# yzqin/s4g-release

Hardware: AMD Instinct MI355X
Metric: scenes/sec (25.6k-pt clouds) end-to-end grasp inference (higher is better)
Workload: dtype f32 (f16x2 split)

## Files before the change

### s4g_release_amd/csrc/mlp_heads.hip

```cpp
#include <stdlib.h>

#include "mlp_common.h"

#ifndef S4G_HEADS_ABLATE
#define S4G_HEADS_ABLATE 0
#endif

namespace s4g {

__device__ __forceinline__ void heads_keep_alive(const f32x16& v) { asm volatile("" ::"v"(v)); }

struct HeadsParams {
  int P, N;
  const float* X;
  int ldx;
  const uint16_t* W[5];
  const float* bias[5];
  const float* wsc[5];
  float* out[4];
  int ch[4];
  long long obs[4];
  int head_mask;
  int sigmoid_head;
  const float* a_amax;
  float a_floor;
  int rps;
  const uint16_t* Wp[2];
  const float* bias_p[2];
  const float* wsc_p[2];
  const int* nidx;
  const float* nw;
  const float* sparse;
  const float* dense;
  const float* lbias;
  const float* a_amax2;
  int N2;
};

template <int PL, int HD_RING, int NRBT, bool PRE>
__global__ __launch_bounds__(512, 2) void mlp_heads_kernel(const HeadsParams p) {
  constexpr int BM = 32 * NRBT, C = 256, NW = 8, astr = C + 8, aplane = BM * astr;
  constexpr int FB = PL * 1024;
  extern __shared__ __attribute__((aligned(16))) float smemf[];
  uint16_t* PA = reinterpret_cast<uint16_t*>(smemf);
  uint16_t* PB = PA + PL * aplane;
  float* scr = reinterpret_cast<float*>(PB + PL * aplane);

  const int t = threadIdx.x;
  const int lane = t & 63;
  const int li = lane & 31, lh = lane >> 5;
  const int wv = __builtin_amdgcn_readfirstlane(t >> 6);
  const int p0 = blockIdx.x * BM;
  const uint32_t wf_lane = (uint32_t)lane * 16u;

  float sa = 1.f, inv_sa = 1.f;
  if constexpr (PL == 2) {
    float amax = p.a_floor;
    if constexpr (PRE) {
      if (p.a_amax) amax += amax_rows(p.a_amax, lane, p0, min(p0 + BM, p.P) - 1, p.rps);
      if (p.a_amax2) amax += amax_rows(p.a_amax2, lane, p0, min(p0 + BM, p.P) - 1, p.rps);
    } else if (p.a_amax) {
      amax = fmaxf(amax, amax_rows(p.a_amax, lane, p0, min(p0 + BM, p.P) - 1, p.rps));
    }
    uint32_t ex = __float_as_uint(amax) >> 23;
    ex = ex < 15u ? 15u : (ex > 240u ? 240u : ex);
    ex = __builtin_amdgcn_readfirstlane(ex);
    sa = __uint_as_float((268u - ex) << 23);
    inv_sa = __uint_as_float((ex - 14u) << 23);
  }

  WRef wrs[5];
#pragma unroll
  for (int L = 0; L < 5; ++L) wrs[L] = wref(p.W[L], 0);
  auto woff = [&](int n32, int nks, int ks) { return (size_t)((n32 * nks + ks) * FB); };
  auto w0 = [&](int g, int h) { return wrs[0] + woff(g * 16 + h * 8 + wv, 16, 0); };
  auto w1 = [&](int g, int h) { return wrs[1] + woff(g * 8 + wv, 32, h * 16); };
  auto w2 = [&](int g) { return wrs[2] + woff(g * 8 + wv, 16, 0); };
  auto w3 = [&](int g) { return wrs[3] + woff(g * 4 + (wv & 3), 16, 0); };
  auto wl = [&](int g) { return wrs[4] + woff(g, 8, 0); };
  auto wload = [&](const WRef& w, uint32_t byte_off, int pl) { return wref_load(w, wf_lane + pl * 1024, byte_off); };
  const WRef wp0 = PRE ? wref(p.Wp[0], woff(wv, 16, 0)) : wrs[0];
  const WRef wp1 = PRE ? wref(p.Wp[1], woff(wv, 16, 0)) : wrs[0];

  const int hmask = p.head_mask;
  const int g_first = __builtin_ctz(hmask);
  uint4 ring[HD_RING][PL];
  {
    const WRef w = PRE ? wp0 : w0(g_first, 0);
#pragma unroll
    for (int d = 0; d < HD_RING; ++d)
#pragma unroll
      for (int pl = 0; pl < PL; ++pl) ring[d][pl] = wload(w, d * FB, pl);
  }

#pragma unroll 1
  for (int r0 = 0; r0 < BM; r0 += 64) {
    const int row = r0 + (t >> 3), chunk = t & 7;
    const bool ok = p0 + row < p.P;
    float4 ra[8];
    if constexpr (PRE) {
      const int pos = ok ? p0 + row : 0;
      const int bq = pos / p.N;
      int i3[3];
      float w3[3];
#pragma unroll
      for (int k = 0; k < 3; ++k) {
        i3[k] = bq * p.N2 + p.nidx[(size_t)pos * 3 + k];
        w3[k] = p.nw[(size_t)pos * 3 + k];
      }
#pragma unroll
      for (int h = 0; h < 2; ++h) {
        float4 a[4], b[4], c[4], y[4], bb[4];
#pragma unroll
        for (int kk = 0; kk < 4; ++kk) {
          const int col = (h * 4 + kk) * 32 + chunk * 4;
          a[kk] = *reinterpret_cast<const float4*>(p.sparse + (size_t)i3[0] * 256 + col);
          b[kk] = *reinterpret_cast<const float4*>(p.sparse + (size_t)i3[1] * 256 + col);
          c[kk] = *reinterpret_cast<const float4*>(p.sparse + (size_t)i3[2] * 256 + col);
          bb[kk] = *reinterpret_cast<const float4*>(p.lbias + col);
          y[kk] = p.dense ? *reinterpret_cast<const float4*>(p.dense + (size_t)pos * 256 + col)
                          : make_float4(0.f, 0.f, 0.f, 0.f);
        }
#pragma unroll
        for (int kk = 0; kk < 4; ++kk) {
          const float av[4] = {a[kk].x, a[kk].y, a[kk].z, a[kk].w}, bv[4] = {b[kk].x, b[kk].y, b[kk].z, b[kk].w};
          const float cv[4] = {c[kk].x, c[kk].y, c[kk].z, c[kk].w}, yv[4] = {y[kk].x, y[kk].y, y[kk].z, y[kk].w};
          const float bi[4] = {bb[kk].x, bb[kk].y, bb[kk].z, bb[kk].w};
          float r[4];
#pragma unroll
          for (int e = 0; e < 4; ++e) {
            float acc = __fmul_rn(av[e], w3[0]);
            acc = __fadd_rn(acc, __fmul_rn(bv[e], w3[1]));
            acc = __fadd_rn(acc, __fmul_rn(cv[e], w3[2]));
            r[e] = ok ? fmaxf(__fadd_rn(__fadd_rn(yv[e], acc), bi[e]), 0.f) : 0.f;
          }
          ra[h * 4 + kk] = make_float4(r[0], r[1], r[2], r[3]);
        }
      }
    } else {
    const float* src = p.X + (size_t)(ok ? p0 + row : 0) * p.ldx + chunk * 4;
#pragma unroll
    for (int kt = 0; kt < 8; ++kt)
      ra[kt] = ok ? nt_load4(src + kt * 32) : make_float4(0.f, 0.f, 0.f, 0.f);
    }
#pragma unroll
    for (int kt = 0; kt < 8; ++kt) {
      uint16_t* dst = PA + row * astr + kt * 32 + chunk * 4;
      if constexpr (PL == 2) {
        uint2 h, l;
        split2_h<false>(ra[kt], sa, h, l);
        *reinterpret_cast<uint2*>(dst) = h;
        *reinterpret_cast<uint2*>(dst + aplane) = l;
      } else {
        *reinterpret_cast<uint2*>(dst) = make_uint2(cvt_pk_bf16(ra[kt].x, ra[kt].y), cvt_pk_bf16(ra[kt].z, ra[kt].w));
      }
    }
  }
  __syncthreads();

#define S4G_HD_TERM(NRB, PA_, PB_, ZERO)                                                            \
  _Pragma("unroll") for (int rb = 0; rb < NRB; ++rb)                                                \
    acc[rb] = chain_mfma<PL>(bf[PB_], af[rb][PA_], (ZERO) ? zero16 : acc[rb]);
#define S4G_HD_STRIP(PANEL, NRB, ROWOFF, WCUR, NKS, WNEXT)                                          \
  {                                                                                                 \
    const uint16_t* a_lane = (PANEL) + ((ROWOFF) + li) * astr + 8 * lh;                             \
    uint4 afn[NRBT][PL];                                                                            \
    _Pragma("unroll") for (int rb = 0; rb < NRB; ++rb) _Pragma("unroll") for (int pl = 0; pl < PL; ++pl) \
      afn[rb][pl] = *reinterpret_cast<const uint4*>(a_lane + pl * aplane + rb * 32 * astr);         \
    const WRef wcur_ = (WCUR);                                                                      \
    const WRef wnext_ = (WNEXT);                                                                    \
    _Pragma("unroll") for (int ks = 0; ks < NKS; ++ks) {                                            \
      const int d = ks % HD_RING;                                                                   \
      const int ksn = ks + 1 == NKS ? 0 : ks + 1;                                                   \
      uint4 af[NRBT][PL], bf[PL];                                                                   \
      _Pragma("unroll") for (int rb = 0; rb < NRB; ++rb) _Pragma("unroll") for (int pl = 0; pl < PL; ++pl) { \
        af[rb][pl] = afn[rb][pl];                                                                   \
        if (!(S4G_HEADS_ABLATE & 2))                                                                \
          afn[rb][pl] = *reinterpret_cast<const uint4*>(a_lane + pl * aplane + rb * 32 * astr + ksn * 16); \
      }                                                                                             \
      _Pragma("unroll") for (int pl = 0; pl < PL; ++pl) bf[pl] = ring[d][pl];                       \
      {                                                                                             \
        const int kr = ks + HD_RING;                                                                \
        _Pragma("unroll") for (int pl = 0; pl < PL; ++pl)                                           \
          if (!(S4G_HEADS_ABLATE & 1))                                                              \
            ring[d][pl] = kr < NKS ? wload(wcur_, kr * FB, pl) : wload(wnext_, (kr - NKS) * FB, pl); \
      }                                                                                             \
      if constexpr (PL == 2) {                                                                      \
        S4G_HD_TERM(NRB, 0, 1, ks == 0)                                                             \
        S4G_HD_TERM(NRB, 1, 0, false)                                                               \
        S4G_HD_TERM(NRB, 0, 0, false)                                                               \
      } else {                                                                                      \
        S4G_HD_TERM(NRB, 0, 0, ks == 0)                                                             \
      }                                                                                             \
      _Pragma("unroll") for (int q = 0; q < PL; ++q) {                                              \
        __builtin_amdgcn_sched_group_barrier(0x008, 1, 0);                                          \
        __builtin_amdgcn_sched_group_barrier(0x020, 1, 0);                                          \
        __builtin_amdgcn_sched_group_barrier(0x008, 1, 0);                                          \
        __builtin_amdgcn_sched_group_barrier(0x100, 1, 0);                                          \
      }                                                                                             \
      __builtin_amdgcn_sched_barrier(0);                                                            \
    }                                                                                               \
  }

  f32x16 zero16;
#pragma unroll
  for (int r = 0; r < 16; ++r) zero16[r] = 0.f;
  f32x16 acc[NRBT];
  float* epi_s = scr + wv * 64;

  auto stage_sb2 = [&](const float* wsc, const float* bias, int gch, float mul) {
    epi_s[lane] = lane < 32 ? (PL == 2 ? mul * wsc[gch + lane] : 1.f) : bias[gch + lane - 32];
  };
  auto stage_sb = [&](int L, int gch, float mul) { stage_sb2(p.wsc[L], p.bias[L], gch, mul); };

  float inv_sh = 1.f;
  auto panel_epilogue_to = [&](uint16_t* PD, auto nrb_tag, int rowoff, int pch0) {
    constexpr int NRB = decltype(nrb_tag)::value;
    if (S4G_HEADS_ABLATE & 4) {
#pragma unroll
      for (int rb = 0; rb < NRB; ++rb) heads_keep_alive(acc[rb]);
      if (!(S4G_HEADS_ABLATE & 8)) {
        __syncthreads();
        __syncthreads();
      }
      return;
    }
    float tmax = 0.f;
#pragma unroll
    for (int j = 0; j < 4; ++j) {
      const float4 sc4 = *reinterpret_cast<const float4*>(epi_s + 8 * j + 4 * lh);
      const float4 b4 = *reinterpret_cast<const float4*>(epi_s + 32 + 8 * j + 4 * lh);
      const float scv[4] = {sc4.x, sc4.y, sc4.z, sc4.w};
      const float bv[4] = {b4.x, b4.y, b4.z, b4.w};
#pragma unroll
      for (int rb = 0; rb < NRB; ++rb) {
        const f32x2 x01 = pk_fma(f32x2{acc[rb][4 * j], acc[rb][4 * j + 1]}, f32x2{scv[0], scv[1]}, f32x2{bv[0], bv[1]});
        const f32x2 x23 = pk_fma(f32x2{acc[rb][4 * j + 2], acc[rb][4 * j + 3]}, f32x2{scv[2], scv[3]}, f32x2{bv[2], bv[3]});
        const float x[4] = {fmaxf(x01.x, 0.f), fmaxf(x01.y, 0.f), fmaxf(x23.x, 0.f), fmaxf(x23.y, 0.f)};
#pragma unroll
        for (int e = 0; e < 4; ++e) acc[rb][4 * j + e] = x[e];
        if constexpr (PL == 2) {
          tmax = fmaxf(fmaxf(tmax, x[0]), x[1]);
          tmax = fmaxf(fmaxf(tmax, x[2]), x[3]);
        }
      }
    }
    float sh = 1.f;
    if constexpr (PL == 2) {
      const uint32_t wm = wave_max_u32(__float_as_uint(tmax));
      if (lane == 0) scr[NW * 64 + wv] = __uint_as_float(wm);
    }
    __syncthreads();
    if constexpr (PL == 2) {
      float hmax = scr[NW * 64];
#pragma unroll
      for (int w = 1; w < NW; ++w) hmax = fmaxf(hmax, scr[NW * 64 + w]);
      uint32_t exh = __float_as_uint(hmax) >> 23;
      exh = exh < 15u ? 15u : (exh > 240u ? 240u : exh);
      exh = __builtin_amdgcn_readfirstlane(exh);
      sh = __uint_as_float((268u - exh) << 23);
      inv_sh = __uint_as_float((exh - 14u) << 23);
    }
#pragma unroll
    for (int j = 0; j < 4; ++j)
#pragma unroll
      for (int rb = 0; rb < NRB; ++rb) {
        uint16_t* dst = PD + (rowoff + rb * 32 + li) * astr + pch0 + 8 * j + 4 * lh;
        if constexpr (PL == 2) {
          const float4 v = make_float4(acc[rb][4 * j], acc[rb][4 * j + 1], acc[rb][4 * j + 2], acc[rb][4 * j + 3]);
          uint2 h, l;
          split2_h<false>(v, sh, h, l);
          *reinterpret_cast<uint2*>(dst) = h;
          *reinterpret_cast<uint2*>(dst + aplane) = l;
        } else {
          *reinterpret_cast<uint2*>(dst) = make_uint2(cvt_pk_bf16(acc[rb][4 * j], acc[rb][4 * j + 1]),
                                                      cvt_pk_bf16(acc[rb][4 * j + 2], acc[rb][4 * j + 3]));
        }
      }
    __syncthreads();
  };
  auto panel_epilogue = [&](auto nrb_tag, int rowoff, int pch0) { panel_epilogue_to(PB, nrb_tag, rowoff, pch0); };
  using full = std::integral_constant<int, NRBT>;
  using half = std::integral_constant<int, NRBT / 2>;

  if constexpr (PRE) {
    stage_sb2(p.wsc_p[0], p.bias_p[0], wv * 32, inv_sa);
    S4G_HD_STRIP(PA, NRBT, 0, wp0, 16, wp1)
    panel_epilogue(full{}, 0, wv * 32);
    stage_sb2(p.wsc_p[1], p.bias_p[1], wv * 32, inv_sh);
    S4G_HD_STRIP(PB, NRBT, 0, wp1, 16, w0(g_first, 0))
    panel_epilogue_to(PA, full{}, 0, wv * 32);
    inv_sa = inv_sh;
  }

  for (int g = g_first, gn; g >= 0; g = gn) {
    const int rest = hmask >> (g + 1);
    gn = rest ? g + 1 + __builtin_ctz(rest) : -1;
    const int gnx = gn >= 0 ? gn : g;
    f32x16 acc1[NRBT];
    stage_sb(0, g * 512 + wv * 32, inv_sa);
    S4G_HD_STRIP(PA, NRBT, 0, w0(g, 0), 16, w1(g, 0))
    panel_epilogue(full{}, 0, wv * 32);
    S4G_HD_STRIP(PB, NRBT, 0, w1(g, 0), 16, w0(g, 1))
#pragma unroll
    for (int rb = 0; rb < NRBT; ++rb)
#pragma unroll
      for (int r = 0; r < 16; r += 2) {
        const f32x2 v = f32x2{acc[rb][r], acc[rb][r + 1]} * f32x2{inv_sh, inv_sh};
        acc1[rb][r] = v.x;
        acc1[rb][r + 1] = v.y;
      }
    stage_sb(0, g * 512 + 256 + wv * 32, inv_sa);
    S4G_HD_STRIP(PA, NRBT, 0, w0(g, 1), 16, w1(g, 1))
    panel_epilogue(full{}, 0, wv * 32);
    S4G_HD_STRIP(PB, NRBT, 0, w1(g, 1), 16, w2(g))
#pragma unroll
    for (int rb = 0; rb < NRBT; ++rb)
#pragma unroll
      for (int r = 0; r < 16; r += 2) {
        const f32x2 v = pk_fma(f32x2{acc[rb][r], acc[rb][r + 1]}, f32x2{inv_sh, inv_sh}, f32x2{acc1[rb][r], acc1[rb][r + 1]});
        acc[rb][r] = v.x;
        acc[rb][r + 1] = v.y;
      }
    stage_sb(1, g * 256 + wv * 32, 1.f);
    panel_epilogue(full{}, 0, wv * 32);
    stage_sb(2, g * 256 + wv * 32, inv_sh);
    S4G_HD_STRIP(PB, NRBT, 0, w2(g), 16, w3(g))
    panel_epilogue(full{}, 0, wv * 32);
    {
      const int row3 = (wv >> 2) * (BM / 2), cg = wv & 3;
      stage_sb(3, g * 128 + cg * 32, inv_sh);
      const WRef after = wv < NRBT ? wl(g) : w0(gnx, 0);
      S4G_HD_STRIP(PB, NRBT / 2, row3, w3(g), 16, after)
      panel_epilogue(half{}, row3, cg * 32);
    }
    if (wv < NRBT) {
      stage_sb(4, g * 32, inv_sh);
      S4G_HD_STRIP(PB, 1, wv * 32, wl(g), 8, w0(gnx, 0))
      const int row = p0 + wv * 32 + li;
      const int b = row / p.N, pt = row - b * p.N;
      const int nch = p.ch[g];
      float* __restrict__ base = p.out[g] + (size_t)b * (size_t)p.obs[g] + pt;
#pragma unroll
      for (int j = 0; j < 4; ++j) {
        const float4 sc4 = *reinterpret_cast<const float4*>(epi_s + 8 * j + 4 * lh);
        const float4 b4 = *reinterpret_cast<const float4*>(epi_s + 32 + 8 * j + 4 * lh);
        const float scv[4] = {sc4.x, sc4.y, sc4.z, sc4.w};
        const float bv[4] = {b4.x, b4.y, b4.z, b4.w};
#pragma unroll
        for (int e = 0; e < 4; ++e) {
          const int c = 8 * j + 4 * lh + e;
          float x = __fmaf_rn(acc[0][4 * j + e], scv[e], bv[e]);
          if (g == p.sigmoid_head) x = 1.0f / (1.0f + expf(-x));
          if (c < nch && row < p.P) base[(size_t)c * p.N] = x;
        }
      }
    }
  }
#undef S4G_HD_STRIP
#undef S4G_HD_TERM
}

template <int PL, int HD_RING, int NRBT, bool PRE>
static int launch_heads_cfg(const HeadsParams& p, hipStream_t st) {
  constexpr int BM = 32 * NRBT;
  constexpr size_t lds = sizeof(uint16_t) * 2 * PL * BM * (256 + 8) + sizeof(float) * (8 * 64 + 16);
  static_assert(lds <= 160 * 1024, "one workgroup's panels must fit a CU's LDS");
  static LdsAttrCache lds_cache;
  if (int rc = allow_dynamic_lds(reinterpret_cast<const void*>(&mlp_heads_kernel<PL, HD_RING, NRBT, PRE>), lds, lds_cache)) return rc;
  hipLaunchKernelGGL((mlp_heads_kernel<PL, HD_RING, NRBT, PRE>), dim3((unsigned)((p.P + BM - 1) / BM)), dim3(512), lds, st, p);
  S4G_LAUNCH_CHECK();
  return S4G_OK;
}
template <int PL, int HD_RING, int NRBT>
static int launch_heads(const HeadsParams& p, hipStream_t st) {
  return p.Wp[0] ? launch_heads_cfg<PL, HD_RING, NRBT, true>(p, st) : launch_heads_cfg<PL, HD_RING, NRBT, false>(p, st);
}

}

extern "C" int s4g_heads_chain_f32(const s4g_heads_desc_t* d, s4g_stream_t stream) {
  using namespace s4g;
  if (!d || d->P < 0 || d->N <= 0) return S4G_EINVAL;
  const bool pre = d->pre_W_frag[0] != nullptr;
  if (!pre && (!d->X || (d->ldx & 3) || d->ldx < 256 || ((uintptr_t)d->X & 15))) return S4G_EINVAL;
  if (pre && (!d->pre_W_frag[1] || !d->pre_bias[0] || !d->pre_bias[1] || !d->pre_nidx || !d->pre_nw ||
              !d->pre_sparse || !d->pre_lbias || d->pre_N2 < 3 || ((uintptr_t)d->pre_sparse & 15) ||
              ((uintptr_t)d->pre_dense & 15) || ((uintptr_t)d->pre_lbias & 15) ||
              (d->precision == S4G_GEMM_F16X2 && (!d->pre_w_inv_scale[0] || !d->pre_w_inv_scale[1]))))
    return S4G_EINVAL;
  if (d->precision != S4G_GEMM_F16X2 && d->precision != S4G_GEMM_BF16) return S4G_EINVAL;
  if (d->C != 256 || d->H0 != 512 || d->H1 != 256 || d->H2 != 256 || d->H3 != 128) return S4G_EUNSUPPORTED;
  HeadsParams p;
  p.P = d->P;
  p.N = d->N;
  p.X = d->X;
  p.ldx = d->ldx;
  for (int l = 0; l < 5; ++l) {
    if (!d->W_frag[l] || !d->bias[l] || (d->precision == S4G_GEMM_F16X2 && !d->w_inv_scale[l])) return S4G_EINVAL;
    p.W[l] = (const uint16_t*)d->W_frag[l];
    p.bias[l] = d->bias[l];
    p.wsc[l] = d->w_inv_scale[l];
  }
  p.head_mask = d->head_mask ? d->head_mask : 15;
  if (p.head_mask < 0 || p.head_mask > 15) return S4G_EINVAL;
  for (int h = 0; h < 4; ++h) {
    p.out[h] = nullptr;
    p.ch[h] = 0;
    p.obs[h] = 0;
    if (!((p.head_mask >> h) & 1)) continue;
    if (!d->out[h] || d->channels[h] <= 0 || d->channels[h] > 32) return S4G_EINVAL;
    p.out[h] = d->out[h];
    p.ch[h] = d->channels[h];
    if (d->out_batch_stride != 0 && d->out_batch_stride < (int64_t)d->channels[h] * d->N) return S4G_EINVAL;
    p.obs[h] = d->out_batch_stride != 0 ? (long long)d->out_batch_stride : (long long)d->channels[h] * d->N;
  }
  p.sigmoid_head = d->sigmoid_head;
  p.a_amax = d->a_amax;
  p.a_floor = d->a_amax_floor;
  p.rps = d->rows_per_scene > 0 ? d->rows_per_scene : 0;
  for (int l = 0; l < 2; ++l) {
    p.Wp[l] = pre ? (const uint16_t*)d->pre_W_frag[l] : nullptr;
    p.bias_p[l] = pre ? d->pre_bias[l] : nullptr;
    p.wsc_p[l] = pre ? d->pre_w_inv_scale[l] : nullptr;
  }
  p.nidx = pre ? d->pre_nidx : nullptr;
  p.nw = pre ? d->pre_nw : nullptr;
  p.sparse = pre ? d->pre_sparse : nullptr;
  p.dense = pre ? d->pre_dense : nullptr;
  p.lbias = pre ? d->pre_lbias : nullptr;
  p.a_amax2 = pre ? d->pre_a_amax2 : nullptr;
  p.N2 = pre ? d->pre_N2 : 0;
  if (d->precision == S4G_GEMM_F16X2 && !d->a_amax && !(d->a_amax_floor > 0.f)) return S4G_EINVAL;
  if (d->P == 0) return S4G_OK;
  hipStream_t st = (hipStream_t)stream;
  if (d->precision == S4G_GEMM_F16X2) return launch_heads<2, 4, 2>(p, st);
  return launch_heads<1, 4, 4>(p, st);
}
```

Baseline: 1993.

## Use 16x16x32 f16 MFMA tiles with swizzled LDS panels in split-precision heads

For the two-plane (f16 hi/lo split) path, the heads kernel now uses 16x16x32 MFMA instructions instead of the 32-wide chained MFMA. Weight fragments are re-indexed per lane and activations are read through a new XOR-swizzled LDS layout with a wider row pad. Explicit sched_group_barrier hints interleave LDS reads, weight loads and MFMAs. The accumulator layout, epilogue and output store are generalized to match. This aims to reduce LDS bank conflicts and improve MFMA issue, at the cost of more LDS usage and more complex fragment bookkeeping.

Result: no change. 2005, median of 6 (+0.6%).

```diff
diff --git a/s4g_release_amd/csrc/mlp_heads.hip b/s4g_release_amd/csrc/mlp_heads.hip
--- a/s4g_release_amd/csrc/mlp_heads.hip
+++ b/s4g_release_amd/csrc/mlp_heads.hip
@@ -37,9 +37,46 @@
   int N2;
 };
 
+__device__ __forceinline__ void heads_keep_alive(const f32x4& v) { asm volatile("" ::"v"(v)); }
+
+__device__ __forceinline__ f32x4 heads_mfma16(const uint4 a, const uint4 b, const f32x4 c) {
+  return __builtin_amdgcn_mfma_f32_16x16x32_f16(__builtin_bit_cast(f16x8, a), __builtin_bit_cast(f16x8, b), c, 0, 0, 0);
+}
+
+template <int PL, int NRBT>
+struct HeadsAcc {
+  static constexpr int NJ = 4, BPB = 1;
+  f32x16 v[NRBT];
+  __device__ __forceinline__ float get(int b, int j, int e) const { return v[b][4 * j + e]; }
+  __device__ __forceinline__ void set(int b, int j, int e, float x) { v[b][4 * j + e] = x; }
+  __device__ __forceinline__ void keep_alive(int nb) const {
+#pragma unroll
+    for (int b = 0; b < NRBT; ++b)
+      if (b < nb) heads_keep_alive(v[b]);
+  }
+};
+template <int NRBT>
+struct HeadsAcc<2, NRBT> {
+  static constexpr int NJ = 2, BPB = 2;
+  f32x4 v[2][2 * NRBT];
+  __device__ __forceinline__ float get(int b, int j, int e) const { return v[j][b][e]; }
+  __device__ __forceinline__ void set(int b, int j, int e, float x) { v[j][b][e] = x; }
+  __device__ __forceinline__ void keep_alive(int nb) const {
+#pragma unroll
+    for (int b = 0; b < 2 * NRBT; ++b)
+      if (b < nb) {
+        heads_keep_alive(v[0][b]);
+        heads_keep_alive(v[1][b]);
+      }
+  }
+};
+
 template <int PL, int HD_RING, int NRBT, bool PRE>
 __global__ __launch_bounds__(512, 2) void mlp_heads_kernel(const HeadsParams p) {
-  constexpr int BM = 32 * NRBT, C = 256, NW = 8, astr = C + 8, aplane = BM * astr;
+  constexpr int BM = 32 * NRBT, C = 256, NW = 8, astr = C + (PL == 2 ? 16 : 8), aplane = BM * astr;
+  using Acc = HeadsAcc<PL, NRBT>;
+  constexpr int NJ = Acc::NJ, BPB = Acc::BPB;
+  constexpr int RD = PL == 2 ? HD_RING / 2 : HD_RING, RW = PL == 2 ? 4 : 1;
   constexpr int FB = PL * 1024;
   extern __shared__ __attribute__((aligned(16))) float smemf[];
   uint16_t* PA = reinterpret_cast<uint16_t*>(smemf);
@@ -49,9 +86,14 @@
   const int t = threadIdx.x;
   const int lane = t & 63;
   const int li = lane & 31, lh = lane >> 5;
+  const int r16 = lane & 15, q16 = lane >> 4;
+  const int prow = PL == 2 ? r16 : li;
+  const int cho = PL == 2 ? 4 * q16 : 4 * lh;
+  constexpr int CGS = 32 / NJ, PBS = 32 / BPB;
+  auto pcol = [&](int row, int col) { return PL == 2 ? (col ^ (((row >> 2) & 3) << 3)) : col; };
   const int wv = __builtin_amdgcn_readfirstlane(t >> 6);
   const int p0 = blockIdx.x * BM;
-  const uint32_t wf_lane = (uint32_t)lane * 16u;
+  const uint32_t wf_lane = PL == 2 ? (uint32_t)((q16 >> 1) * (PL * 1024) + (32 * (q16 & 1) + r16) * 16) : (uint32_t)lane * 16u;
 
   float sa = 1.f, inv_sa = 1.f;
   if constexpr (PL == 2) {
@@ -79,18 +121,19 @@
   auto w3 = [&](int g) { return wrs[3] + woff(g * 4 + (wv & 3), 16, 0); };
   auto wl = [&](int g) { return wrs[4] + woff(g, 8, 0); };
   auto wload = [&](const WRef& w, uint32_t byte_off, int pl) { return wref_load(w, wf_lane + pl * 1024, byte_off); };
+  auto wload16 = [&](const WRef& w, uint32_t byte_off, int i) { return wref_load(w, wf_lane + (i >> 1) * 256 + (i & 1) * 1024, byte_off); };
   const WRef wp0 = PRE ? wref(p.Wp[0], woff(wv, 16, 0)) : wrs[0];
   const WRef wp1 = PRE ? wref(p.Wp[1], woff(wv, 16, 0)) : wrs[0];
 
   const int hmask = p.head_mask;
   const int g_first = __builtin_ctz(hmask);
-  uint4 ring[HD_RING][PL];
+  uint4 ring[RD][PL * RW];
   {
     const WRef w = PRE ? wp0 : w0(g_first, 0);
 #pragma unroll
-    for (int d = 0; d < HD_RING; ++d)
-#pragma unroll
-      for (int pl = 0; pl < PL; ++pl) ring[d][pl] = wload(w, d * FB, pl);
+    for (int d = 0; d < RD; ++d)
+#pragma unroll
+      for (int i = 0; i < PL * RW; ++i) ring[d][i] = PL == 2 ? wload16(w, d * 2 * FB, i) : wload(w, d * FB, i);
   }
 
 #pragma unroll 1
@@ -145,7 +188,7 @@
     }
 #pragma unroll
     for (int kt = 0; kt < 8; ++kt) {
-      uint16_t* dst = PA + row * astr + kt * 32 + chunk * 4;
+      uint16_t* dst = PA + row * astr + kt * 32 + pcol(row, chunk * 4);
       if constexpr (PL == 2) {
         uint2 h, l;
         split2_h<false>(ra[kt], sa, h, l);
@@ -160,8 +203,53 @@
 
 #define S4G_HD_TERM(NRB, PA_, PB_, ZERO)                                                            \
   _Pragma("unroll") for (int rb = 0; rb < NRB; ++rb)                                                \
-    acc[rb] = chain_mfma<PL>(bf[PB_], af[rb][PA_], (ZERO) ? zero16 : acc[rb]);
+    acc.v[rb] = chain_mfma<PL>(bf[PB_], af[rb][PA_], (ZERO) ? zero16 : acc.v[rb]);
+#define S4G_HD_STRIP16(PANEL, NRB, ROWOFF, WCUR, NKS, WNEXT)                                        \
+  {                                                                                                 \
+    constexpr int NB_ = 2 * (NRB), NS_ = (NKS) / 2;                                                 \
+    const uint16_t* a_lane = (PANEL) + ((ROWOFF) + r16) * astr + pcol(r16, 8 * q16);                \
+    uint4 pf[2 * NRBT][2];                                                                          \
+    _Pragma("unroll") for (int pb = 0; pb < NB_; ++pb) _Pragma("unroll") for (int pl = 0; pl < 2; ++pl) \
+      pf[pb][pl] = *reinterpret_cast<const uint4*>(a_lane + pl * aplane + pb * 16 * astr);          \
+    const WRef wcur_ = (WCUR);                                                                      \
+    const WRef wnext_ = (WNEXT);                                                                    \
+    _Pragma("unroll") for (int ks = 0; ks < NS_; ++ks) {                                            \
+      const int d = ks % RD;                                                                        \
+      const int ksn = ks + 1 == NS_ ? 0 : ks + 1;                                                   \
+      const int kr = ks + RD;                                                                       \
+      uint4 wf[4];                                                                                  \
+      _Pragma("unroll") for (int i = 0; i < 4; ++i) {                                               \
+        wf[i] = ring[d][i];                                                                         \
+        if (!(S4G_HEADS_ABLATE & 1))                                                                \
+          ring[d][i] = kr < NS_ ? wload16(wcur_, kr * 2 * FB, i) : wload16(wnext_, (kr - NS_) * 2 * FB, i); \
+      }                                                                                             \
+      _Pragma("unroll") for (int pb = 0; pb < NB_; ++pb) {                                          \
+        const uint4 ph = pf[pb][0], pl_ = pf[pb][1];                                                \
+        if (!(S4G_HEADS_ABLATE & 2))                                                                \
+          _Pragma("unroll") for (int pl = 0; pl < 2; ++pl)                                          \
+            pf[pb][pl] = *reinterpret_cast<const uint4*>(a_lane + pl * aplane + pb * 16 * astr + ksn * 32); \
+        _Pragma("unroll") for (int h = 0; h < 2; ++h)                                               \
+          acc.v[h][pb] = heads_mfma16(wf[2 * h + 1], ph, ks == 0 ? zero4 : acc.v[h][pb]);           \
+        _Pragma("unroll") for (int h = 0; h < 2; ++h)                                               \
+          acc.v[h][pb] = heads_mfma16(wf[2 * h], pl_, acc.v[h][pb]);                                \
+        _Pragma("unroll") for (int h = 0; h < 2; ++h)                                               \
+          acc.v[h][pb] = heads_mfma16(wf[2 * h], ph, acc.v[h][pb]);                                 \
+      }                                                                                             \
+      _Pragma("unroll") for (int pb = 0; pb < NB_; ++pb) {                                          \
+        __builtin_amdgcn_sched_group_barrier(0x008, 1, 0);                                          \
+        __builtin_amdgcn_sched_group_barrier(0x020, 1, 0);                                          \
+        __builtin_amdgcn_sched_group_barrier(0x008, 2, 0);                                          \
+        __builtin_amdgcn_sched_group_barrier(0x020, NB_ == 2 ? 1 : 0, 0);                           \
+        __builtin_amdgcn_sched_group_barrier(0x008, 3, 0);                                          \
+        __builtin_amdgcn_sched_group_barrier(0x100, 2, 0);                                          \
+      }                                                                                             \
+      __builtin_amdgcn_sched_barrier(0);                                                            \
+    }                                                                                               \
+  }
 #define S4G_HD_STRIP(PANEL, NRB, ROWOFF, WCUR, NKS, WNEXT)                                          \
+  if constexpr (PL == 2) S4G_HD_STRIP16(PANEL, NRB, ROWOFF, WCUR, NKS, WNEXT)                       \
+  else S4G_HD_STRIP32(PANEL, NRB, ROWOFF, WCUR, NKS, WNEXT)
+#define S4G_HD_STRIP32(PANEL, NRB, ROWOFF, WCUR, NKS, WNEXT)                                        \
   {                                                                                                 \
     const uint16_t* a_lane = (PANEL) + ((ROWOFF) + li) * astr + 8 * lh;                             \
     uint4 afn[NRBT][PL];                                                                            \
@@ -205,7 +293,8 @@
   f32x16 zero16;
 #pragma unroll
   for (int r = 0; r < 16; ++r) zero16[r] = 0.f;
-  f32x16 acc[NRBT];
+  f32x4 zero4 = {0.f, 0.f, 0.f, 0.f};
+  Acc acc;
   float* epi_s = scr + wv * 64;
 
   auto stage_sb2 = [&](const float* wsc, const float* bias, int gch, float mul) {
@@ -215,10 +304,9 @@
 
   float inv_sh = 1.f;
   auto panel_epilogue_to = [&](uint16_t* PD, auto nrb_tag, int rowoff, int pch0) {
-    constexpr int NRB = decltype(nrb_tag)::value;
+    constexpr int NB = decltype(nrb_tag)::value * BPB;
     if (S4G_HEADS_ABLATE & 4) {
-#pragma unroll
-      for (int rb = 0; rb < NRB; ++rb) heads_keep_alive(acc[rb]);
+      acc.keep_alive(NB);
       if (!(S4G_HEADS_ABLATE & 8)) {
         __syncthreads();
         __syncthreads();
@@ -227,18 +315,18 @@
     }
     float tmax = 0.f;
 #pragma unroll
-    for (int j = 0; j < 4; ++j) {
-      const float4 sc4 = *reinterpret_cast<const float4*>(epi_s + 8 * j + 4 * lh);
-      const float4 b4 = *reinterpret_cast<const float4*>(epi_s + 32 + 8 * j + 4 * lh);
+    for (int j = 0; j < NJ; ++j) {
+      const float4 sc4 = *reinterpret_cast<const float4*>(epi_s + CGS * j + cho);
+      const float4 b4 = *reinterpret_cast<const float4*>(epi_s + 32 + CGS * j + cho);
       const float scv[4] = {sc4.x, sc4.y, sc4.z, sc4.w};
       const float bv[4] = {b4.x, b4.y, b4.z, b4.w};
 #pragma unroll
-      for (int rb = 0; rb < NRB; ++rb) {
-        const f32x2 x01 = pk_fma(f32x2{acc[rb][4 * j], acc[rb][4 * j + 1]}, f32x2{scv[0], scv[1]}, f32x2{bv[0], bv[1]});
-        const f32x2 x23 = pk_fma(f32x2{acc[rb][4 * j + 2], acc[rb][4 * j + 3]}, f32x2{scv[2], scv[3]}, f32x2{bv[2], bv[3]});
+      for (int rb = 0; rb < NB; ++rb) {
+        const f32x2 x01 = pk_fma(f32x2{acc.get(rb, j, 0), acc.get(rb, j, 1)}, f32x2{scv[0], scv[1]}, f32x2{bv[0], bv[1]});
+        const f32x2 x23 = pk_fma(f32x2{acc.get(rb, j, 2), acc.get(rb, j, 3)}, f32x2{scv[2], scv[3]}, f32x2{bv[2], bv[3]});
         const float x[4] = {fmaxf(x01.x, 0.f), fmaxf(x01.y, 0.f), fmaxf(x23.x, 0.f), fmaxf(x23.y, 0.f)};
 #pragma unroll
-        for (int e = 0; e < 4; ++e) acc[rb][4 * j + e] = x[e];
+        for (int e = 0; e < 4; ++e) acc.set(rb, j, e, x[e]);
         if constexpr (PL == 2) {
           tmax = fmaxf(fmaxf(tmax, x[0]), x[1]);
           tmax = fmaxf(fmaxf(tmax, x[2]), x[3]);
@@ -262,19 +350,19 @@
       inv_sh = __uint_as_float((exh - 14u) << 23);
     }
 #pragma unroll
-    for (int j = 0; j < 4; ++j)
-#pragma unroll
-      for (int rb = 0; rb < NRB; ++rb) {
-        uint16_t* dst = PD + (rowoff + rb * 32 + li) * astr + pch0 + 8 * j + 4 * lh;
+    for (int j = 0; j < NJ; ++j)
+#pragma unroll
+      for (int rb = 0; rb < NB; ++rb) {
+        uint16_t* dst = PD + (rowoff + rb * PBS + prow) * astr + pch0 + pcol(prow, CGS * j + cho);
         if constexpr (PL == 2) {
-          const float4 v = make_float4(acc[rb][4 * j], acc[rb][4 * j + 1], acc[rb][4 * j + 2], acc[rb][4 * j + 3]);
+          const float4 v = make_float4(acc.get(rb, j, 0), acc.get(rb, j, 1), acc.get(rb, j, 2), acc.get(rb, j, 3));
           uint2 h, l;
           split2_h<false>(v, sh, h, l);
           *reinterpret_cast<uint2*>(dst) = h;
           *reinterpret_cast<uint2*>(dst + aplane) = l;
         } else {
-          *reinterpret_cast<uint2*>(dst) = make_uint2(cvt_pk_bf16(acc[rb][4 * j], acc[rb][4 * j + 1]),
-                                                      cvt_pk_bf16(acc[rb][4 * j + 2], acc[rb][4 * j + 3]));
+          *reinterpret_cast<uint2*>(dst) = make_uint2(cvt_pk_bf16(acc.get(rb, j, 0), acc.get(rb, j, 1)),
+                                                      cvt_pk_bf16(acc.get(rb, j, 2), acc.get(rb, j, 3)));
         }
       }
     __syncthreads();
@@ -297,30 +385,33 @@
     const int rest = hmask >> (g + 1);
     gn = rest ? g + 1 + __builtin_ctz(rest) : -1;
     const int gnx = gn >= 0 ? gn : g;
-    f32x16 acc1[NRBT];
+    Acc acc1;
     stage_sb(0, g * 512 + wv * 32, inv_sa);
     S4G_HD_STRIP(PA, NRBT, 0, w0(g, 0), 16, w1(g, 0))
     panel_epilogue(full{}, 0, wv * 32);
     S4G_HD_STRIP(PB, NRBT, 0, w1(g, 0), 16, w0(g, 1))
 #pragma unroll
-    for (int rb = 0; rb < NRBT; ++rb)
-#pragma unroll
-      for (int r = 0; r < 16; r += 2) {
-        const f32x2 v = f32x2{acc[rb][r], acc[rb][r + 1]} * f32x2{inv_sh, inv_sh};
-        acc1[rb][r] = v.x;
-        acc1[rb][r + 1] = v.y;
+    for (int rb = 0; rb < NRBT * BPB; ++rb)
+#pragma unroll
+      for (int r = 0; r < 4 * NJ; r += 2) {
+        const int j = r >> 2, e = r & 3;
+        const f32x2 v = f32x2{acc.get(rb, j, e), acc.get(rb, j, e + 1)} * f32x2{inv_sh, inv_sh};
+        acc1.set(rb, j, e, v.x);
+        acc1.set(rb, j, e + 1, v.y);
       }
     stage_sb(0, g * 512 + 256 + wv * 32, inv_sa);
     S4G_HD_STRIP(PA, NRBT, 0, w0(g, 1), 16, w1(g, 1))
     panel_epilogue(full{}, 0, wv * 32);
     S4G_HD_STRIP(PB, NRBT, 0, w1(g, 1), 16, w2(g))
 #pragma unroll
-    for (int rb = 0; rb < NRBT; ++rb)
-#pragma unroll
-      for (int r = 0; r < 16; r += 2) {
-        const f32x2 v = pk_fma(f32x2{acc[rb][r], acc[rb][r + 1]}, f32x2{inv_sh, inv_sh}, f32x2{acc1[rb][r], acc1[rb][r + 1]});
-        acc[rb][r] = v.x;
-        acc[rb][r + 1] = v.y;
+    for (int rb = 0; rb < NRBT * BPB; ++rb)
+#pragma unroll
+      for (int r = 0; r < 4 * NJ; r += 2) {
+        const int j = r >> 2, e = r & 3;
+        const f32x2 v = pk_fma(f32x2{acc.get(rb, j, e), acc.get(rb, j, e + 1)}, f32x2{inv_sh, inv_sh},
+                               f32x2{acc1.get(rb, j, e), acc1.get(rb, j, e + 1)});
+        acc.set(rb, j, e, v.x);
+        acc.set(rb, j, e + 1, v.y);
       }
     stage_sb(1, g * 256 + wv * 32, 1.f);
     panel_epilogue(full{}, 0, wv * 32);
@@ -337,34 +428,39 @@
     if (wv < NRBT) {
       stage_sb(4, g * 32, inv_sh);
       S4G_HD_STRIP(PB, 1, wv * 32, wl(g), 8, w0(gnx, 0))
-      const int row = p0 + wv * 32 + li;
-      const int b = row / p.N, pt = row - b * p.N;
       const int nch = p.ch[g];
-      float* __restrict__ base = p.out[g] + (size_t)b * (size_t)p.obs[g] + pt;
-#pragma unroll
-      for (int j = 0; j < 4; ++j) {
-        const float4 sc4 = *reinterpret_cast<const float4*>(epi_s + 8 * j + 4 * lh);
-        const float4 b4 = *reinterpret_cast<const float4*>(epi_s + 32 + 8 * j + 4 * lh);
-        const float scv[4] = {sc4.x, sc4.y, sc4.z, sc4.w};
-        const float bv[4] = {b4.x, b4.y, b4.z, b4.w};
-#pragma unroll
-        for (int e = 0; e < 4; ++e) {
-          const int c = 8 * j + 4 * lh + e;
-          float x = __fmaf_rn(acc[0][4 * j + e], scv[e], bv[e]);
-          if (g == p.sigmoid_head) x = 1.0f / (1.0f + expf(-x));
-          if (c < nch && row < p.P) base[(size_t)c * p.N] = x;
+#pragma unroll
+      for (int pb = 0; pb < BPB; ++pb) {
+        const int row = p0 + wv * 32 + pb * PBS + prow;
+        const int b = row / p.N, pt = row - b * p.N;
+        float* __restrict__ base = p.out[g] + (size_t)b * (size_t)p.obs[g] + pt;
+#pragma unroll
+        for (int j = 0; j < NJ; ++j) {
+          const float4 sc4 = *reinterpret_cast<const float4*>(epi_s + CGS * j + cho);
+          const float4 b4 = *reinterpret_cast<const float4*>(epi_s + 32 + CGS * j + cho);
+          const float scv[4] = {sc4.x, sc4.y, sc4.z, sc4.w};
+          const float bv[4] = {b4.x, b4.y, b4.z, b4.w};
+#pragma unroll
+          for (int e = 0; e < 4; ++e) {
+            const int c = CGS * j + cho + e;
+            float x = __fmaf_rn(acc.get(pb, j, e), scv[e], bv[e]);
+            if (g == p.sigmoid_head) x = 1.0f / (1.0f + expf(-x));
+            if (c < nch && row < p.P) base[(size_t)c * p.N] = x;
+          }
         }
       }
     }
   }
 #undef S4G_HD_STRIP
+#undef S4G_HD_STRIP16
+#undef S4G_HD_STRIP32
 #undef S4G_HD_TERM
 }
 
 template <int PL, int HD_RING, int NRBT, bool PRE>
 static int launch_heads_cfg(const HeadsParams& p, hipStream_t st) {
   constexpr int BM = 32 * NRBT;
-  constexpr size_t lds = sizeof(uint16_t) * 2 * PL * BM * (256 + 8) + sizeof(float) * (8 * 64 + 16);
+  constexpr size_t lds = sizeof(uint16_t) * 2 * PL * BM * (256 + (PL == 2 ? 16 : 8)) + sizeof(float) * (8 * 64 + 16);
   static_assert(lds <= 160 * 1024, "one workgroup's panels must fit a CU's LDS");
   static LdsAttrCache lds_cache;
   if (int rc = allow_dynamic_lds(reinterpret_cast<const void*>(&mlp_heads_kernel<PL, HD_RING, NRBT, PRE>), lds, lds_cache)) return rc;
```
